# iucario/WorkoutDetector

Hardware: AMD Instinct MI355X
Metric: clips/sec (8x3x224x224 TSM-R50) (higher is better)
Workload: dtype f32; 1 GPU; TSM-R50 8-seg 224x224 12-class inference, batch 32 clips per GPU, f32 NHWC, device-resident input (BASELINE.json configs[1]); clips_per_gpu=32, num_segments=8, height=224, width=224, num_class=12, weights=seeded random init (no trained weights offline), parallelism=single GPU

## Files before the change

workoutdetector_amd/csrc/tsm_conv_rules.h:

```cpp
#pragma once
#include <stdint.h>
#include <string.h>

#if defined(__HIPCC__)
#define TSM_HOST_DEVICE __host__ __device__
#else
#define TSM_HOST_DEVICE
#endif

namespace tsm {

struct ConvParams {
  const float *x;
  const float *w;
  const float *bias;
  const float *res;
  float *y;
  int N, Hi, Wi, C, logC4;
  int Ho, Wo, Cout;
  int stride, pad;
  int Kp;
  int M;
  int relu;
  int T;
  int fold;
  int ntm, ntn;
  int tile;
  int prec;
  const float *x2;
  int C2, Hi2, Wi2, stride2;
  int K1;
  int kseg_len;
  int ksplit;
  int tail_from;
  float *ypart;
  int reverse;
  int pos_major;
};

enum ConvPrec { kPrecF32 = 0, kPrecBf16x3 = 1, kPrecBf16 = 2 };
constexpr int kPrecBlockShift = 4;
constexpr int kPrecPosMajor = 8;

enum ConvTile {
  kTileAuto = 0, kTile128x128 = 1, kTile128x64 = 2, kTile64x64 = 3, kTile32x32 = 4,
  kTile128x128w8 = 5,
  kTile256x256 = 6,
  kTileWs = 7,
  kTile256x256p = 8,
  kNumTiles = 9
};

struct Fused23Params {
  const float *x;
  const float *w2;
  const float *bias2;
  const float *w3f;
  const float *bias3;
  const float *res;
  float *y;
// ... 288 lines not shown
    case kTile256x256p:
      return p.prec == kPrecBf16 && p.Cout % 256 == 0 && p.C % 64 == 0 && !(p.res && p.x2) && (p.pad != 1 || (!p.res && p.T == 0)) &&
             (!p.x2 || (p.K1 % 64 == 0 && p.C2 % 64 == 0)) && (tile == kTile256x256 || (p.Cout <= 2048 && p.Kp >= 128));
    case kTileWs: {
      int tr, tc;
      return conv3x3_ws_valid(p, &tr, &tc) || conv3x3_ws128s2_valid(p, &tr, &tc) || conv3x3_ws128_valid(p, &tr, &tc, nullptr) ||
             conv1x1_ws_valid(p) || conv1x1_wsn_valid(p, n_cu);
    }
    default: return false;
  }
}

enum ConvFamily { kFamInvalid = 0, kFamIgemm, kFamIgemmSeg, kFamBf16_256, kFamBf16_256p, kFamWs3x3, kFamWs128, kFamWs128s2, kFamWs1x1, kFamWsn };

struct ConvRoute {
  int family = kFamInvalid, ks = 0;
  int bm = 0, bn = 0, wgm = 0, wgn = 0;
  bool shift = false, res = false, dual = false, block_shift = false;
  bool pos_major = false;
  int ntm = 0, ntn = 0;
  long tiles = 0;
  unsigned grid = 0;
  int tr = 0, tc = 0, swz = 0;
};

inline bool conv_args_refused(const ConvParams &p, int ks) {
  const int kc = p.prec == kPrecBf16 ? 64 : kBK;
  if (p.Cout % 64 != 0 || p.Kp % kc != 0 || p.M <= 0) return true;
  if (p.logC4 < 0 || p.logC4 > 28 || (1 << p.logC4) * 4 != p.C) return true;
  if (ks != 7 && p.C % kc != 0) return true;
  if (p.T > 0 && ((ks != 1 && ks != 3) || (ks == 3 && p.kseg_len > 0) || p.N % p.T != 0 || p.fold % 4 != 0 ||
                  (p.res && 2 * (int64_t)p.fold > p.Cout) || (p.x2 && 2 * (int64_t)p.fold > p.C2)))
    return true;
  if (p.x2 && (ks != 1 || p.res || p.K1 % kc != 0 || p.C2 % kc != 0 || (int64_t)p.K1 + p.C2 != p.Kp || p.K1 != p.C))
    return true;
  if (p.x2 && (128.0 / ((double)p.Ho * p.Wo) + 4.0) * (double)p.Hi2 * p.Wi2 * p.C2 * 4.0 > 2.0e9) return true;
  if (p.T > 0 && p.res && (128.0 + 2.0 * p.Ho * p.Wo) * p.Cout * 4.0 > 2.0e9) return true;
  if (p.prec != kPrecF32 && p.prec != kPrecBf16x3 && p.prec != kPrecBf16) return true;
  if (p.kseg_len < 0 || (p.kseg_len > 0 && (p.prec != kPrecF32 || p.res || ks == 7))) return true;
  if ((p.ksplit && p.kseg_len <= 0) || p.ksplit < 0 || p.ksplit > 2) return true;
  if (p.prec != kPrecF32 && p.T > 0 && p.fold % 8 != 0) return true;
  if (ks == 7 && (p.C != 4 || (p.prec != kPrecF32 && (p.stride != 2 || p.pad != 3)))) return true;
  if ((128.0 / ((double)p.Ho * p.Wo) + 4.0) * (double)p.Hi * p.Wi * p.C * 4.0 > 2.0e9) return true;
  return (ks != 1 && ks != 3 && ks != 7) || (ks == 7 && p.res);
}

// ... 8 lines not shown
  for (int ky = 0; ky < 3; ++ky)
    for (int kx = 0; kx < 3; ++kx)
      if ((unsigned)(iy0 + ky) < (unsigned)Hi && (unsigned)(ix0 + kx) < (unsigned)Wi) mask |= 1u << (ky * 3 + kx);
  return mask;
}
TSM_HOST_DEVICE inline int next_live_kstep(int kt, unsigned mask, int steps_per_tap, int nk) {
  if (kt < 0 || kt >= nk) return nk;
  const int log_spt = __builtin_ctz((unsigned)steps_per_tap);
  const int tap = kt >> log_spt;
  const unsigned rest = tap < 9 ? (mask & 0x1ffu) >> tap : 0u;
  if (rest & 1u) return kt;
  if (rest == 0u) return nk;
  const int next = (tap + __builtin_ctz(rest)) << log_spt;
  return next < nk ? next : nk;
}
inline bool pos_major_valid(const ConvParams &p, int ks) {
  return p.prec == kPrecF32 && ks == 3 && p.pad == 1 && (p.stride == 1 || p.stride == 2) && p.kseg_len > 0 && p.T == 0 &&
         !p.res && !p.x2 && (p.tile == kTile64x64 || p.tile == kTileAuto) && (p.ksplit == 0 || p.ksplit == 2) &&
         p.N > 0 && p.N % 64 == 0 && p.Ho > 0 && p.Wo > 0 && (int64_t)p.N * p.Ho * p.Wo == p.M &&
         p.C >= kBK && (p.C & (p.C - 1)) == 0 && p.Kp == (int64_t)9 * p.C &&
         (double)p.N * p.Hi * p.Wi * p.C * 4.0 < 2.0e9 && (double)p.M * p.Cout * 4.0 < 2.0e9;
}

inline ConvRoute conv_route(const ConvParams &p, int ks, int n_cu) {
  ConvRoute r, refused;
  if (conv_args_refused(p, ks) || (p.tile != kTileAuto && !conv_tile_valid(p, p.tile, n_cu))) return refused;
  r.ks = ks; r.res = p.res != nullptr; r.dual = p.x2 != nullptr;
  r.shift = !r.res && p.T > 0 && !(ks == 1 && r.dual);
  if (p.tile == kTileAuto) conv_tile_shape(p, &r.bm, &r.bn);
  else conv_tile_dims(p.tile, &r.bm, &r.bn);
  if (p.tile == kTile256x256 || p.tile == kTile256x256p) {
    const bool persistent = p.tile == kTile256x256p;
    if (!(persistent ? conv_bf16_256p_valid(p, ks) : conv_bf16_256_valid(p, ks))) return refused;
    r.family = persistent ? kFamBf16_256p : kFamBf16_256;
    r.wgm = 2; r.wgn = 4;
    r.shift = ks == 1 && p.T > 0;
    r.ntm = (int)(((long)p.M + 255) / 256); r.ntn = p.Cout / 256;
    r.tiles = (long)r.ntm * r.ntn;
    const int slots = n_cu & ~7;
    r.grid = (unsigned)(!persistent || r.tiles < slots || slots < 8 ? r.tiles : slots);
    return r.tiles > 0x7fffffffL ? refused : r;
  }
  if (p.tile == kTileWs) {
    if (ks == 3) {
      r.family = conv3x3_ws128s2_valid(p, &r.tr, &r.tc) ? kFamWs128s2 : conv3x3_ws128_valid(p, &r.tr, &r.tc, &r.swz) ? kFamWs128 :
                 conv3x3_ws_valid(p, &r.tr, &r.tc) ? kFamWs3x3 : kFamInvalid;
// ... 11 lines not shown
      const int pairs = n_cu >> 4 << 3;
      r.grid = 2u * (unsigned)(r.tiles < pairs ? (r.tiles + 7) / 8 * 8 : pairs);
    }
    return r;
  }
  if (p.kseg_len > 0 && r.bm != 32) r.bm = r.bn = 64;
  if (r.bm == 32 && p.prec != kPrecF32) return refused;
  r.wgm = r.bm == 32 ? 1 : r.bm == 128 && r.bn == 128 && p.tile == kTile128x128w8 ? 4 : 2;
  r.wgn = r.bm == 32 ? 1 : 2;
  r.ntm = (int)(((long)p.M + r.bm - 1) / r.bm); r.ntn = p.Cout / r.bn;
  r.tiles = (long)r.ntm * r.ntn;
  long grid = r.tiles;
  if (p.kseg_len > 0) {
    if (r.res || ks == 7 || (r.shift && ks == 3)) return refused;
    if (p.ksplit == 2 && (p.tail_from <= 0 || p.tail_from >= r.tiles || p.tail_from % r.ntn != 0)) return refused;
    r.family = kFamIgemmSeg;
    r.pos_major = p.pos_major != 0 && r.bm == 64 && pos_major_valid(p, ks);
    grid = p.ksplit == 2 ? p.tail_from + (r.tiles - p.tail_from) * conv_num_segments(p) : r.tiles * (p.ksplit ? conv_num_segments(p) : 1);
  } else {
    r.family = kFamIgemm;
  }
  r.block_shift = p.T > 0 && (r.dual || r.res);
  r.grid = (unsigned)grid;
  return grid > 0x7fffffffL ? refused : r;
}

inline bool conv23_ws_valid(int n, int h, int w, int *tr_out = nullptr, int *tc_out = nullptr) {
  int tr, tc;
  return n > 0 && h > 0 && w > 0 && (double)h * w * 512.0 < 2.0e9 && (double)n * h * w < 2.0e9 &&
         ws_tile_geometry(h, w, tr_out ? tr_out : &tr, tc_out ? tc_out : &tc);
}
inline bool bneck_ws_valid(int cin, int n, int h, int w, int T, int fold) {
  return (cin == 256 || cin == 64) && n > 0 && h > 0 && w >= 1 && w <= 64 && (double)h * w * 512.0 * 3.0 < 2.0e9 &&
         (T == 0 || (T > 0 && n % T == 0 && fold == cin / 8));
}
inline bool front_s2_valid(int n, int h, int w, int T, int fold) {
  return n > 0 && h >= 2 && (h & 1) == 0 && w >= 2 && w <= 64 && (double)h * w * 512.0 * 3.0 < 2.0e9 &&
         (T == 0 || (T > 0 && n % T == 0 && fold == 32));
}
inline int conv31_rows(const Conv31Params &p) {
  if (p.K3 == 128 && p.C == 512 && p.N1 == 128) return 256;
  if ((p.K3 == 128 && p.C == 512 && p.N1 == 256) || (p.K3 == 256 && p.C == 1024 && p.N1 == 256)) return 128;
  return 0;
}
inline bool conv31_valid(const Conv31Params &p) {
  const int m = conv31_rows(p);
  if (m == 0) return false;
// ... 7 lines not shown
```

workoutdetector_amd/csrc/tsm_engine.hip:

```cpp
#include <hip/hip_runtime.h>

#include <sys/stat.h>

#include <algorithm>
#include <cerrno>
#include <cmath>
#include <cstdio>
#include <cstdlib>
#include <cstring>
#include <map>
#include <string>
#include <vector>

#include "../../include/tsm_hip.h"
#include "tsm_host_util.h"
#include "tsm_kernels.h"

#ifndef TSM_BUILD_ID
#define TSM_BUILD_ID __DATE__ "/" __TIME__
#endif

namespace {

using namespace tsm_host;
// ... 151 lines not shown
  float *d_in4 = nullptr;
  float *buf[5] = {nullptr, nullptr, nullptr, nullptr, nullptr};
  float *d_pooled = nullptr, *d_logits = nullptr;
  float *d_partial = nullptr;
  size_t partial_elems = 0;
  size_t buf_elems = 0;
  int h1 = 0, w1 = 0, hp = 0, wp = 0;
  hipEvent_t ev0 = nullptr, ev1 = nullptr;
  bool have_time = false;
  std::vector<void *> allocs;
  bool poison = false;
  std::vector<GuardBuf> guards;
  std::map<int, std::vector<int>> tile_cache;
  bool autotune = true;
  bool stem_pool = true;
  bool stem_direct = true;
  bool stem_planar = true;
  std::string tune_path, tune_sig;
  int force_tile = 0, force_code = -1;
  int fuse23 = -1;
  int fuse_block = -1;
  int fuse31 = -1;
  int fuse_front = -1;
  bool pos_major = true;
  int walk = -1;
  int n_cu = 256;
  int timing_left = 0;
  bool timing_only3x3 = false;
  std::vector<std::vector<hipEvent_t>> timing;
  std::vector<hipEvent_t> event_pool;
  std::vector<hipEvent_t> *cur_timing = nullptr;
};

namespace {

int fail(tsm_engine *e, int code, const std::string &msg) {
  if (e) e->err = msg; else g_create_error = msg;
  return code;
}

#define TSM_HIP(e, call)                                                                        \
  do {                                                                                          \
    hipError_t _st = (call);                                                                    \
    if (_st != hipSuccess)                                                                      \
      return fail((e), TSM_ERR_HIP, std::string(#call) + ": " + hipGetErrorString(_st));        \
  } while (0)
// ... 320 lines not shown
  fclose(f);
  return ok;
}

void tune_cache_store(tsm_engine *e, int key, const std::vector<int> &codes) {
  if (e->tune_path.empty()) return;
  std::string line = e->tune_sig + "|" + std::to_string(key) + "|";
  for (size_t i = 0; i < codes.size(); ++i) line += (i ? "," : "") + std::to_string(codes[i]);
  line += "\n";
  if (line.size() >= 4096) return;
  FILE *f = fopen(e->tune_path.c_str(), "a");
  if (!f) return;
  fwrite(line.data(), 1, line.size(), f);
  fclose(f);
}

bool tail_split_from(const tsm::ConvParams &p, int n_cu, size_t partial_elems, int *tail_from) {
  if (p.kseg_len <= 0) return false;
  const long from = tsm_host::tail_split_point(p.M, p.Cout, tsm::conv_num_segments(p), n_cu, partial_elems);
  *tail_from = (int)from;
  return from > 0;
}

hipError_t launch_conv_code(tsm::ConvParams p, int ks, int code, float *partial, size_t partial_elems, int n_cu, hipStream_t s) {
  p.tile = code & kCodeTileMask;
  const bool pos_major = (code & kCodePosMajor) && !(code & kCodeSplitK) && (code & kCodeTileMask) == tsm::kTile64x64 &&
                         tsm::pos_major_valid(p, ks);
  p.pos_major = pos_major ? 1 : 0;
  if ((code & kCodeSplitK) && p.kseg_len > 0 &&
      (size_t)tsm::conv_num_segments(p) * (size_t)p.M * (size_t)p.Cout <= partial_elems) {
    float *y = p.y;
    p.ksplit = 1;
    p.y = partial;
    hipError_t st = tsm::launch_conv(p, ks, s);
    if (st == hipSuccess)
      st = tsm::launch_splitk_reduce(partial, tsm::conv_num_segments(p), p.M, p.Cout, p.bias, nullptr, y, p.relu, s);
    return st;
  }
  if ((code & kCodeTailK) && (code & kCodeTileMask) == tsm::kTile64x64 && p.kseg_len > 0) {
    int tail_from = 0;
    if (tail_split_from(p, n_cu, partial_elems, &tail_from)) {
      float *y = p.y;
      const int mt0 = tail_from / (p.Cout / 64) * 64;
      p.ksplit = 2;
      p.tail_from = tail_from;
      p.ypart = partial;
      hipError_t st = tsm::launch_conv(p, ks, s);
      if (st == hipSuccess && pos_major)
        st = tsm::launch_splitk_reduce_pos(partial, tsm::conv_num_segments(p), mt0, p.M - mt0, p.N, p.Ho * p.Wo, p.Cout, p.bias, y,
                                           p.relu, s);
      else if (st == hipSuccess)
        st = tsm::launch_splitk_reduce(partial, tsm::conv_num_segments(p), p.M - mt0, p.Cout, p.bias, nullptr,
                                       y + (size_t)mt0 * p.Cout, p.relu, s);
      return st;
    }
  }
  return tsm::launch_conv(p, ks, s);
}

int checked_code(const tsm::ConvParams &p, int code, int n_cu) {
  return code > 0 && (code & ~kCodeValid) == 0 && tsm::conv_tile_valid(p, code & kCodeTileMask, n_cu) ? code : 0;
}

struct Tap {
  const float *ptr = nullptr;
  int64_t shape[4] = {0, 0, 0, 0};
  bool hit = false;
};

struct LaunchTimer {
  tsm_engine *e;
  hipStream_t s;
  bool on;
  bool skip;
  LaunchTimer(tsm_engine *e_, hipStream_t s_, bool is3x3)
      : e(e_), s(s_), on(e_->cur_timing != nullptr), skip(e_->timing_only3x3 && !is3x3) { mark(); }
  ~LaunchTimer() { mark(); }
  void mark() {
    if (!on) return;
    if (skip) {
      e->cur_timing->push_back(nullptr);
      return;
    }
    hipEvent_t ev = nullptr;
// ... 175 lines not shown
    int rc = time_best_of(e, s, many, &many_ms);
    if (!rc) rc = time_best_of(e, s, one, &one_ms);
    *wins = one_ms < many_ms;
    return rc;
  }
  int conv(int idx, tsm::ConvParams p, int ks, bool is3x3);
  int run_basic(size_t k, int nn, float *x, float *y, int hh, int ww);
  int run_block(size_t k, const BlockPlan &plan, int nn, float *x, float *y, int hh, int ww);
  int run_nonlocal(size_t k, int nn, float *x, float *z, int hh, int ww);
  int run_mse(size_t k, int nn, int hh, int ww);
  int tune_block(size_t k, int nn, float *x, float *y, int hh, int ww);
};

hipError_t Forward::launch_code(tsm::ConvParams p, int ks, int code) {
  return launch_conv_code(p, ks, code, e->d_partial, e->partial_elems, e->n_cu, s);
}

int Forward::conv(int idx, tsm::ConvParams p, int ks, bool is3x3) {
  p.reverse = next_dir();
  if (!tuning) {
    int code = tiles ? (*tiles)[idx] : 0;
    if (e->force_tile) code = e->force_tile;
    if (e->force_code >= 0) code = e->force_code;
    TSM_LAUNCH_K(e, s, is3x3, launch_code(p, ks, checked_code(p, code, e->n_cu)));
    return TSM_OK;
  }
  std::vector<int> cands;
  if (p.kseg_len > 0) {
    const size_t need = (size_t)tsm::conv_num_segments(p) * p.M * p.Cout;
    const long tiles64 = (long)((p.M + 63) / 64) * (p.Cout / 64);
    for (int t : {(int)tsm::kTile64x64, (int)tsm::kTile32x32}) {
      cands.push_back(t);
      if (need <= e->partial_elems && tiles64 < 4L * e->n_cu) cands.push_back(t | kCodeSplitK);
    }
    int tail_from = 0;
    const bool tail = tail_split_from(p, e->n_cu, e->partial_elems, &tail_from);
    if (tail) cands.push_back((int)tsm::kTile64x64 | kCodeTailK);
    tsm::ConvParams q = p;
    q.tile = tsm::kTile64x64;
    if (e->pos_major && tsm::pos_major_valid(q, ks)) {
      cands.push_back((int)tsm::kTile64x64 | kCodePosMajor);
      if (tail) cands.push_back((int)tsm::kTile64x64 | kCodePosMajor | kCodeTailK);
    }
  } else {
    for (int t = 1; t < tsm::kNumTiles; ++t)
      if (tsm::conv_tile_valid(p, t, e->n_cu)) cands.push_back(t);
  }
  float best_ms = 0.f;
  int best = 0;
  for (int t : cands) {
    float ms = 0.f;
    const int rc = time_best_of(e, s, [&] { return launch_code(p, ks, t); }, &ms);
    if (rc) return rc;
    if (best == 0 || ms < best_ms) {
      best = t;
      best_ms = ms;
    }
  }
  (*tiles)[idx] = best;
  return TSM_OK;
}

int Forward::run_basic(size_t k, int nn, float *x, float *y, int hh, int ww) {
  const Block &blk = e->blocks[k];
  const std::string &name = blk.name;
  const ConvLayer &c1 = e->convs[blk.conv1], &c2 = e->convs[blk.conv2];
  const int T = blk.T, shiftT = e->cfg.is_shift ? T : 0;
  const int ho = conv_out_size(hh, 3, blk.stride), wo = conv_out_size(ww, 3, blk.stride);
  const float *identity = x;
// ... 876 lines not shown
  }
  if (cfg->shift_div <= 0 || (64 % cfg->shift_div) != 0 || (64 / cfg->shift_div) % 4 != 0)
    return fail(nullptr, TSM_ERR_UNSUPPORTED, "shift_div must divide 64 with fold % 4 == 0 (8 or 16... )");
  if (prec_of_dtype(cfg->dtype) < 0)
    return fail(nullptr, TSM_ERR_UNSUPPORTED, "dtype must be TSM_DTYPE_F32, TSM_DTYPE_BF16X3 or TSM_DTYPE_BF16");
  if (cfg->dtype != TSM_DTYPE_F32 && (64 / cfg->shift_div) % 8 != 0)
    return fail(nullptr, TSM_ERR_UNSUPPORTED, "the bf16 formats need fold % 8 == 0 (shift_div <= 8)");
  int ndev = 0;
  hipError_t st = hipGetDeviceCount(&ndev);
  if (st != hipSuccess || ndev <= 0)
    return fail(nullptr, TSM_ERR_HIP, std::string("no HIP device: ") + hipGetErrorString(st));
  if (cfg->device_id < 0 || cfg->device_id >= ndev) return fail(nullptr, TSM_ERR_INVALID_ARG, "bad device_id");
  tsm_engine *e = new tsm_engine();
  e->cfg = *cfg;
  e->prec = prec_of_dtype(cfg->dtype);
  const auto on = [](const char *s) { return atoi(s) != 0; };
  env_read("TSM_AUTOTUNE", &e->autotune, on);
  env_read("TSM_STEM_DIRECT", &e->stem_direct, on);
  env_read("TSM_STEM_POOL", &e->stem_pool, on);
  env_read("TSM_STEM_PLANAR", &e->stem_planar, on);
  env_read("TSM_CONV_TILE", &e->force_tile, tsm::conv_tile_from_name);
  env_read("TSM_CONV_CODE", &e->force_code, atoi);
  env_read("TSM_POS_MAJOR", &e->pos_major, on);
  env_read("TSM_FUSE_CONV23", &e->fuse23, on);
  env_read("TSM_FUSE_BLOCK", &e->fuse_block, on);
  env_read("TSM_FUSE_C3C1", &e->fuse31, on);
  env_read("TSM_FUSE_FRONT", &e->fuse_front, on);
  env_read("TSM_WALK", &e->walk, on);
  env_read("TSM_POISON", &e->poison, on);
  const char *tc = getenv("TSM_TUNE_CACHE");
  if (!tc) e->tune_path = default_tune_cache_path();
  else if (*tc && strcmp(tc, "0") != 0 && strcmp(tc, "off") != 0) e->tune_path = tc;
  build_topology(e);
  st = hipSetDevice(cfg->device_id);
  if (st == hipSuccess) st = hipStreamCreateWithFlags(&e->stream, hipStreamNonBlocking);
  if (st == hipSuccess) st = hipDeviceGetAttribute(&e->n_cu, hipDeviceAttributeMultiprocessorCount, cfg->device_id);
  if (st == hipSuccess) st = hipEventCreate(&e->ev0);
  if (st == hipSuccess) st = hipEventCreate(&e->ev1);
  if (st != hipSuccess) {
    g_create_error = std::string("engine init: ") + hipGetErrorString(st);
    delete e;
    return TSM_ERR_HIP;
  }
  if (!e->tune_path.empty()) {
    hipDeviceProp_t prop;
    e->tune_sig = "abi" + std::to_string(TSM_ABI_VERSION) + " build " TSM_BUILD_ID " " +
                  (hipGetDeviceProperties(&prop, cfg->device_id) == hipSuccess ? std::string(prop.gcnArchName) : "?") +
                  " cu" + std::to_string(e->n_cu) +
                  " T" + std::to_string(cfg->num_segments) + " " + std::to_string(cfg->height) + "x" +
                  std::to_string(cfg->width) + " dtype" + std::to_string(cfg->dtype) + " shift" +
                  std::to_string(cfg->is_shift ? cfg->shift_div : 0) + " fuse" + std::to_string(e->fuse23) + "/" + std::to_string(e->fuse_block) + "/" + std::to_string(e->fuse31) + "/" + std::to_string(e->fuse_front) +
                  " stem" + std::to_string(e->stem_direct ? 1 : 0) +
                  std::to_string(e->stem_pool ? 1 : 0) + std::to_string(e->stem_planar ? 1 : 0);
    e->tune_sig_base = e->tune_sig.size();
  }
  *out = e;
  return TSM_OK;
}

int tsm_set_backbone(tsm_engine *e, int32_t depth) {
  if (int rc = check_before_weights(e, "tsm_set_backbone")) return rc;
  if (int rc = refuse_on_convnext(e, "tsm_set_backbone")) return rc;
  if (!find_backbone(depth)) return fail(e, TSM_ERR_UNSUPPORTED, "depth must be 18, 34 or 50");
  if (find_backbone(depth)->basic && e->width != 64)
    return fail(e, TSM_ERR_UNSUPPORTED, "a BasicBlock backbone (depth 18 / 34) has no bottleneck width: the engine's is " +
                                            std::to_string(e->width));
  if (find_backbone(depth)->basic && e->non_local)
    return fail(e, TSM_ERR_UNSUPPORTED, "non-local blocks need a Bottleneck backbone (depth 50)");
  e->depth = depth;
  e->backbone_set = 1;
  build_topology(e);
  retag_tune_sig(e);
  return TSM_OK;
}

int tsm_set_bottleneck_width(tsm_engine *e, int32_t width_per_group) {
// ... 457 lines not shown
  };
  const float *xin = a->x, *x2in = a->x2, *rin = a->residual;
  float *yout = a->y, *d_x4 = nullptr, *d_ys = nullptr, *d_part = nullptr;
  if (pl.stem) {
    if ((rc = scratch.alloc(&d_x4, "d_x4", n * in_px * 8, in_px * 8))) return rc;
    TSM_HIP(nullptr, tsm::launch_pack_input(a->x, d_x4, n, hi, wi, 0, prec, s));
    xin = d_x4;
  } else if (x3 && (rc = staged(a->x, "d_xs", (size_t)pl.x_elems, in_px * a->cin, &xin))) {
    return rc;
  }
  if (x3) {
    if ((rc = scratch.alloc(&d_ys, "d_ys", out_elems, out_frame, act_bytes))) return rc;
    yout = d_ys;
    if (rin && (rc = staged(rin, "d_rs", out_elems, out_frame, &rin))) return rc;
    if (pl.dual && (rc = staged(x2in, "d_x2s", (size_t)pl.x2_elems, (size_t)a->hi2 * a->wi2 * a->cin2, &x2in))) return rc;
  }
  tsm::ConvParams p = make_params(c, xin, rin, yout, n, hi, wi, a->relu != 0, pl.T, 1, prec);
  p.fold = pl.fold;
  p.reverse = a->reverse != 0;
  if (pl.dual) set_second_source(&p, c2.kp, x2in, a->cin2, a->hi2, a->wi2, a->stride2);
  int dev = 0, n_cu = 256;
  TSM_HIP(nullptr, hipGetDevice(&dev));
  TSM_HIP(nullptr, hipDeviceGetAttribute(&n_cu, hipDeviceAttributeMultiprocessorCount, dev));
  const int code = checked_code(p, a->code > 0 ? a->code & ~kCodeOpSegmented : a->code, n_cu);
  size_t part_elems = 0;
  if ((code & (kCodeSplitK | kCodeTailK)) && p.kseg_len > 0) {
    part_elems = (size_t)tsm::conv_num_segments(p) * p.M * p.Cout;
    if ((rc = scratch.alloc(&d_part, "d_part", part_elems, out_frame))) return rc;
  }
  const char *sd_env = getenv("TSM_STEM_DIRECT");
  hipError_t st;
  if (pl.stem && x3 && cout == 64 && !(sd_env && atoi(sd_env) == 0))
    st = tsm::launch_stem_direct(xin, c.d_w, c.d_b, yout, n, hi, wi, c.kp, a->relu != 0, prec, s);
  else
    st = launch_conv_code(p, a->k, code, d_part, part_elems, n_cu, s);
  if (st == hipSuccess && x3) st = tsm::launch_to_f32(d_ys, a->y, (int64_t)out_elems / 8, prec, s);
  const hipError_t st2 = hipStreamSynchronize(s);
  if (st != hipSuccess) return op_status("launch_conv", st);
  if (st2 != hipSuccess) return fail(nullptr, TSM_ERR_HIP, std::string("conv sync: ") + hipGetErrorString(st2));
  for (int i = 0; i < scratch.n; ++i) {
    std::string msg;
    TSM_HIP(nullptr, guard_verify(scratch.g[i], &msg));
    if (!msg.empty()) return fail(nullptr, TSM_ERR_GUARD, "tsm_conv_op: " + msg);
  }
  return TSM_OK;
}

// ... 228 lines not shown
```

workoutdetector_amd/csrc/tsm_host_util.h:

```cpp
#pragma once
#include <cmath>
#include <cstddef>
#include <cstdint>
#include <cstdio>
#include <cstdlib>
#include <cstring>
#include <string>
#include <vector>

#include "../../include/tsm_hip.h"
#include "tsm_conv_rules.h"

namespace tsm_host {

constexpr float kBnEps = 1e-5f;
using tsm::kPrecF32;
using tsm::kPrecBf16x3;
using tsm::kPrecBf16;

inline int segment_len(int kp, int prec) {
  if (prec != kPrecF32) return 0;
  const int nk = kp / 32;
  if (nk < 32) return 0;
  const int nseg = nk / 16;
// ... 803 lines not shown
    for (int wn = 0; wn < wgn; ++wn)
      for (int kq = 0; kq < nkq; ++kq)
        for (int lane = 0; lane < 64; ++lane) {
          const int n = j * cmid + wn * 32 + (lane & 31), k0 = 16 * kq + 8 * (lane >> 5);
          const size_t base = ((((size_t)j * wgn + wn) * (2 * nkq) + 2 * kq) * 64 + lane) * 8;
          for (int e = 0; e < 8; ++e) {
            const float x = w3p[(size_t)n * cmid + k0 + e];
            const uint16_t hi = f2bf(x);
            o[base + e] = hi;
            o[base + 64 * 8 + e] = f2bf(x - bf2f(hi));
          }
        }
}

constexpr int kCodeTileMask = 0xF;
constexpr int kCodePosMajor = 0x80;
constexpr int kCodeSplitK = 0x100;
constexpr int kCodeTailK = 0x200;
constexpr int kCodeConv23 = 0x400;
constexpr int kCodeBlock = 0x800;
constexpr int kCodeConv31 = 0x1000;
constexpr int kCodeFront = 0x2000;
constexpr int kCodeFused = kCodeConv23 | kCodeBlock | kCodeConv31 | kCodeFront;
constexpr int kCodeValid = kCodeTileMask | kCodePosMajor | kCodeSplitK | kCodeTailK | kCodeFused;
static_assert((kCodeOpSegmented & kCodeValid) == 0, "the per-op segmented bit must stay clear of the engine's code bits");

inline bool parse_tune_line(const char *line, const std::string &want, int num_tiles, std::vector<int> *codes) {
  if (strncmp(line, want.c_str(), want.size()) != 0) return false;
  std::vector<int> got;
  const char *q = line + want.size();
  while (*q && *q != '\n') {
    char *end = nullptr;
    const long v = strtol(q, &end, 10);
    if (end == q) return false;
    if (v < 0 || (v & ~(long)kCodeValid) != 0 || (int)(v & kCodeTileMask) >= num_tiles) return false;
    got.push_back((int)v);
    if (*end == ',') q = end + 1;
    else if (*end == '\n' || *end == 0) q = end;
    else return false;
  }
  if (got.size() != codes->size()) return false;
  *codes = got;
  return true;
}

}
```

workoutdetector_amd/csrc/tsm_igemm.hip:

```cpp
#include "tsm_device.h"

namespace tsm {

template <int BM, int BN, int WGM, int WGN, int KS, bool SHIFT, bool RES, int PREC, bool DUAL = false, bool SEG = false>
__global__ void __launch_bounds__(64 * WGM * WGN, (SEG && BM == 64) ? ((PREC & kPrecBlockShift) ? 4 : 5) : 1)
conv_igemm(const ConvParams p) {
  constexpr bool BSHIFT = (PREC & kPrecBlockShift) != 0;
  constexpr bool POSM = (PREC & kPrecPosMajor) != 0;
  constexpr int PMODE = PREC & ~(kPrecBlockShift | kPrecPosMajor);
  static_assert(!POSM || (SEG && KS == 3 && BM == 64 && BN == 64 && !SHIFT && !RES && !DUAL && !BSHIFT && PMODE == kPrecF32),
                "position-major rows: the segmented fp32 3x3 on 64x64 tiles only (pos_major_valid)");
  static_assert(!BSHIFT || (!SHIFT && !RES), "block placement: a shifted identity (DUAL = false) or a shifted second source");
  constexpr bool RESID = RES || (BSHIFT && !DUAL);
  static_assert(!SEG || (PMODE == kPrecF32 && !RES && WGM * WGN <= 4 && BM == BN && BM <= 64),
                "segmented K accumulation: fp32, 64x64 / 32x32 tiles, no residual (ConvParams::kseg_len)");
  static_assert(WGM * WGN == 4 || WGM * WGN == 1 || WGM * WGN == 8,
                "4 waves per workgroup, 1 (32x32 small-M tiles) or 8 (128x128 with 4 waves per SIMD at 2 workgroups/CU)");
  constexpr int NT = 64 * WGM * WGN;
  constexpr int LRP = NT / 8;
  static_assert(!DUAL || (KS == 1 && !SHIFT && !RES), "K-concatenated second source: plain 1x1 convs only");
  constexpr bool X3 = PMODE == kPrecBf16x3;
  constexpr bool BF = PMODE == kPrecBf16;
  constexpr int EB = BF ? 2 : 4;
  constexpr int KC = 128 / EB;
  static_assert(!SHIFT || KS == 1 || (KS == 3 && !SEG), "the temporal shift is fused into 1x1 and unsegmented 3x3 convs only");
  constexpr int WTM = BM / WGM, WTN = BN / WGN;
  constexpr int TM = WTM / 32, TN = WTN / 32;
  constexpr int APASS = BM / LRP, BPASS = BN / LRP;
  constexpr bool RK = PMODE == kPrecF32 && ((BM == 64 && BN == 64) || (BM == 32 && BN == 32));
  constexpr int NBUF = RK ? 1 : 2;
  constexpr int CLD = BN + 4;
  static_assert(TM >= 1 && TN >= 1, "wave tile must hold at least one 32x32 MFMA tile");
  constexpr int SMEM_FLOATS = NBUF * (BM + BN) * kLds > BM * CLD ? NBUF * (BM + BN) * kLds : BM * CLD;

  __shared__ __attribute__((aligned(16))) float smem[SMEM_FLOATS];

  const int tid = threadIdx.x;
  const int lane = tid & 63;
  const int wave = tid >> 6;
  const int wm = wave / WGN, wn = wave % WGN;
  const int half = lane >> 5, l31 = lane & 31;

  const int bid = blockIdx.x;
  const bool tail_mode = SEG && p.ksplit == 2;
  const bool in_tail = tail_mode && bid >= p.tail_from;
  const int nwg = tail_mode ? p.tail_from : (int)gridDim.x;
  const int q = nwg >> 3, r = nwg & 7, xcd = bid & 7;
  int tile = (xcd < r ? xcd * (q + 1) : r * (q + 1) + (xcd - r) * q) + (bid >> 3);
  if (p.reverse) tile = nwg - 1 - tile;
  int seg = 0;
  if (SEG && p.ksplit == 1) {
    seg = tile / (p.ntm * p.ntn);
    tile -= seg * (p.ntm * p.ntn);
  }
  if (in_tail) {
    const int u = bid - p.tail_from, n_tail = p.ntm * p.ntn - p.tail_from;
    seg = u / n_tail;
    tile = p.tail_from + (u - seg * n_tail);
  }
  const bool split_wg = SEG && (p.ksplit == 1 || in_tail);
  const int tm = tile / p.ntn, tn = tile - tm * p.ntn;
  const int m0 = tm * BM, n0 = tn * BN;

  const int HoWo = p.Ho * p.Wo;
  const int n_first = POSM ? 0 : m0 / HoWo;
  const int frame0 = SHIFT ? (n_first > 0 ? n_first - 1 : 0) : n_first;
  constexpr bool PAIRS = KS == 7 && PMODE != kPrecF32;
  const int wpairs = (p.Wi + 1) >> 1;
  const size_t frame_elems = PAIRS ? (size_t)p.Hi * wpairs * 8 : (size_t)p.Hi * p.Wi * p.C;
  const size_t a_bytes = ((size_t)p.N - frame0) * frame_elems * EB;
  const __amdgpu_buffer_rsrc_t rsrcA = buffer_window(reinterpret_cast<const char *>(p.x) + (size_t)frame0 * frame_elems * EB, a_bytes);
  const __amdgpu_buffer_rsrc_t rsrcB = buffer_fixed(reinterpret_cast<const char *>(p.w) + (size_t)n0 * p.Kp * EB, BN * p.Kp * EB);

  const size_t frame_elems2 = DUAL ? (size_t)p.Hi2 * p.Wi2 * p.C2 : 0;
  const int frame02 = (BSHIFT && DUAL && n_first > 0) ? n_first - 1 : n_first;
  const size_t a2_bytes = DUAL ? ((size_t)p.N - frame02) * frame_elems2 * EB : 0;
  const __amdgpu_buffer_rsrc_t rsrcA2 = buffer_window(reinterpret_cast<const char *>(DUAL ? p.x2 : p.x) + (size_t)frame02 * frame_elems2 * EB, a2_bytes);

  const int lrow = tid >> 3;
  const int chunk = tid & 7;
  const int frame_bytes = (int)(frame_elems * EB);
  unsigned a_off[APASS];
  unsigned a_offp[SHIFT ? APASS : 1], a_offm[SHIFT ? APASS : 1];
  unsigned a_mask[(KS == 3 && !POSM) ? APASS : 1];
// ... 636 lines not shown
  if constexpr (RES && !SHIFT && KS != 7) {
    if (r.block_shift) TSM_LAUNCH_IGEMM_AND_RETURN(TSM_ARM_RES_SHIFT);
  }
  TSM_LAUNCH_IGEMM_AND_RETURN(TSM_ARM_PLAIN);
}

template <int KS, bool SHIFT, bool RES>
static hipError_t launch_conv_ks(const ConvParams &p, const ConvRoute &r, hipStream_t s) {
  if (r.bm == 32) return launch_conv_t<32, 32, 1, 1, KS, SHIFT, RES>(p, r, s);
  if (r.bm == 128 && r.bn == 128 && r.wgm == 4) return launch_conv_t<128, 128, 4, 2, KS, SHIFT, RES>(p, r, s);
  if (r.bm == 128 && r.bn == 128) return launch_conv_t<128, 128, 2, 2, KS, SHIFT, RES>(p, r, s);
  if (r.bm == 128) return launch_conv_t<128, 64, 2, 2, KS, SHIFT, RES>(p, r, s);
  return launch_conv_t<64, 64, 2, 2, KS, SHIFT, RES>(p, r, s);
}

hipError_t launch_conv(const ConvParams &p_in, int ks, hipStream_t s) {
  const bool device = p_in.tile == kTile256x256 || p_in.tile == kTile256x256p || p_in.tile == kTileWs;
  const DeviceInfo *di = device ? &device_info() : nullptr;
  const ConvRoute r = conv_route(p_in, ks, di ? di->n_cu : 0);
  if (r.family == kFamInvalid) return hipErrorInvalidValue;
  if (di && di->status != hipSuccess) return di->status;
  ConvParams p = p_in;
  p.ntm = r.ntm; p.ntn = r.ntn;
  if (r.family == kFamBf16_256 || r.family == kFamBf16_256p) return launch_conv_bf16_256(p, r, s);
  if (r.family >= kFamWs3x3) return launch_conv_ws(p, r, s);
  if (p.ksplit == 2 && !p.ypart) return hipErrorInvalidValue;
  if (ks == 1) return r.res ? launch_conv_ks<1, false, true>(p, r, s) : r.shift ? launch_conv_ks<1, true, false>(p, r, s) : launch_conv_ks<1, false, false>(p, r, s);
  if (ks == 3) return r.res ? launch_conv_ks<3, false, true>(p, r, s) : r.shift ? launch_conv_ks<3, true, false>(p, r, s) : launch_conv_ks<3, false, false>(p, r, s);
  return launch_conv_ks<7, false, false>(p, r, s);
}

__global__ void __launch_bounds__(256) splitk_reduce_kernel(const float *__restrict__ partial, int n_seg, int64_t n4,
                                                            int64_t seg_stride4, int cout4,
                                                            const float *__restrict__ bias, const float *__restrict__ res,
                                                            float *__restrict__ y, int relu) {
  const int64_t stride = (int64_t)gridDim.x * blockDim.x;
  const float floor_ = relu ? 0.f : -INFINITY;
  const f32x4 *p4 = reinterpret_cast<const f32x4 *>(partial);
  for (int64_t i = (int64_t)blockIdx.x * blockDim.x + threadIdx.x; i < n4; i += stride) {
    f32x4 t = p4[i];
    for (int sgm = 1; sgm < n_seg; ++sgm) t += p4[i + sgm * seg_stride4];
    f32x4 v = t + reinterpret_cast<const f32x4 *>(bias)[i % cout4];
    if (res) v += reinterpret_cast<const f32x4 *>(res)[i];
    v[0] = fmaxf(v[0], floor_);
    v[1] = fmaxf(v[1], floor_);
    v[2] = fmaxf(v[2], floor_);
// ... 50 lines not shown
```

workoutdetector_amd/engine.py:

```python
from __future__ import annotations

import ctypes as C
from dataclasses import dataclass
from typing import Dict, List, Mapping, Optional, Sequence

import numpy as np

from . import _lib
from .weights import (BACKBONES, CONVNEXT, CONVNEXT_DEPTHS, CONVNEXT_WIDTHS, DEPTHS, NL_BLOCKS, SHIFT_PLACES, TDN, TDN_FRAMES, WIDTHS,
                      _convnext_depths, _tdn_depths, feature_width, is_convnext, is_mmaction_state_dict, make_state_dict, make_tdn_state_dict,
                      remap_checkpoint_keys, remap_mmaction_keys, remap_tdn_keys, remap_timm_keys, remap_torchvision_keys, tdn_alpha_beta)

CONSENSUS_TYPES = {'avg': 0, 'identity': 1}


@dataclass
class NodeArg:
    name: str
    shape: list
    type: str = 'tensor(float)'


def _as_f32(a) -> np.ndarray:
    return np.ascontiguousarray(np.asarray(a), dtype=np.float32)
# ... 466 lines not shown
        for li, nb in enumerate(blocks, start=1):
            for b in range(nb):
                p = f'layer{li}.{b}'
                if kind == 'basic':
                    names += ([p + '.downsample'] if b == 0 and li > 1 else []) + [p + '.conv1', p + '.conv2']
                else:
                    names += ([p + '.downsample'] if b == 0 else []) + [p + '.conv1', p + '.conv2', p + '.conv3']
                    if self.non_local and (li, b) in NL_BLOCKS:
                        names += [p + '.nl.qkv', p + '.nl.pool', p + '.nl.attn', p + '.nl.W']
            if self.temporal_pool and li == 1:
                names.append('layer2.tpool')
        return names + ['head']

    @property
    def tdn_chunk_clips(self) -> int:
        per_clip = (self.height // 4) * (self.width // 4) * self.num_segments * 1024
        return max(1, min(8, self.max_clips, ((1 << 29) - 1) // per_clip))

    TILE_NAMES = {0: 'heuristic', 1: '128x128', 2: '128x64', 3: '64x64', 4: '32x32', 5: '128x128w8', 6: '256x256', 7: 'ws',
                  8: '256x256p'}

    @classmethod
    def tile_name(cls, code: int) -> str:
        return (cls.TILE_NAMES[code & 15] + ('/pos' if code & 0x80 else '') + ('/splitK' if code & 0x100 else '') + ('/tailK' if code & 0x200 else '') + ('+conv3' if code & 0x400 else '') +
                ('+block' if code & 0x800 else '') + ('+conv1' if code & 0x1000 else '') + ('+conv2' if code & 0x2000 else ''))

    def conv_tiles(self, n_clips: int) -> Dict[str, str]:
        buf = (C.c_int32 * 256)()
        n = C.c_int32()
        _lib.check(self._lib.tsm_conv_tiles(self._h, n_clips, buf, 256, C.byref(n)), self._h)
        if self.tdn_depths:
            names = ['conv1', 'diff.conv1_5'] + [k for k in self.launch_names() if k.startswith(('resnext_layer1.', 'layer'))
                                                 and k.endswith(('.downsample', '.conv1', '.conv2', '.conv3'))]
            assert n.value == len(names)
            return {k: self.tile_name(buf[i]) for i, k in enumerate(names)}
        if self.convnext_depths:
            names = [k for k in self.launch_names() if k == 'stem.conv' or k.endswith(('.downsample', '.fc1', '.fc2'))]
            assert n.value == len(names)
            return {k: self.tile_name(buf[i]) for i, k in enumerate(names)}
        names = [k for k in self.launch_names() if k not in ('pack_input', 'maxpool', 'head', 'layer2.tpool') and not k.endswith(('.nl.pool', '.nl.attn'))]
        assert n.value == len(names)
        return {k: self.tile_name(buf[i]) for i, k in enumerate(names)}

    def set_layer_timing(self, n_forwards: int, only_conv3x3: bool = False) -> None:
        _lib.check(self._lib.tsm_set_layer_timing(self._h, n_forwards, int(only_conv3x3)), self._h)

    def layer_times_ms(self, forward_index: int) -> Dict[str, float]:
# ... 672 lines not shown
```

Before: 1870 clips/s.

## Add XCD-blocked tile ordering and pos-major frame grouping as autotune candidates

Adds a tile-to-workgroup mapping that splits the output tile grid into 2D blocks per XCD, so each XCD's L2 holds only a slice of the weight columns instead of the full weight matrix. It also adds an optional row remap for the pos-major path that interleaves frame groups. Both are new bits in the tuning code. The autotuner adds them as candidates only when a byte model predicts fewer L2 misses. The cost is a more complex index calculation and more autotune candidates.

After: 1867 clips/s. Within noise of the previous version (-0.2%).

```diff
diff --git a/workoutdetector_amd/csrc/tsm_conv_rules.h b/workoutdetector_amd/csrc/tsm_conv_rules.h
--- a/workoutdetector_amd/csrc/tsm_conv_rules.h
+++ b/workoutdetector_amd/csrc/tsm_conv_rules.h
@@ -36,6 +36,8 @@
   float *ypart;
   int reverse;
   int pos_major;
+  int xcd_n;
+  int pm_group;
 };
 
 enum ConvPrec { kPrecF32 = 0, kPrecBf16x3 = 1, kPrecBf16 = 2 };
@@ -370,6 +372,8 @@
   long tiles = 0;
   unsigned grid = 0;
   int tr = 0, tc = 0, swz = 0;
+  int n_whole = 0, xcd_n = 1;
+  bool pm_group = false;
 };
 
 inline bool conv_args_refused(const ConvParams &p, int ks) {
@@ -424,6 +428,53 @@
          (double)p.N * p.Hi * p.Wi * p.C * 4.0 < 2.0e9 && (double)p.M * p.Cout * 4.0 < 2.0e9;
 }
 
+constexpr int kXcds = 8;
+constexpr long kXcdL2Bytes = 4L << 20;
+constexpr long kXcdSlabMaxBytes = kXcdL2Bytes / 8 * 5;
+
+TSM_HOST_DEVICE inline int xcd_tile_contiguous(int bid, int n_whole, int reverse) {
+  const int q = n_whole >> 3, r = n_whole & 7, xcd = bid & 7;
+  const int tile = (xcd < r ? xcd * (q + 1) : r * (q + 1) + (xcd - r) * q) + (bid >> 3);
+  return reverse ? n_whole - 1 - tile : tile;
+}
+TSM_HOST_DEVICE inline bool xcd_blocks_equal(int ntm, int ntn, int n_whole, int xcd_n) {
+  if (xcd_n != 2 && xcd_n != 4 && xcd_n != 8) return false;
+  if (ntm <= 0 || ntn <= 0 || n_whole <= 0 || n_whole % ntn != 0 || ntn % xcd_n != 0) return false;
+  const int rows = n_whole / ntn;
+  return (rows <= ntm || rows % ntm == 0) && rows % (kXcds / xcd_n) == 0;
+}
+TSM_HOST_DEVICE inline int xcd_tile(int bid, int ntm, int ntn, int n_whole, int xcd_n, int reverse) {
+  if (!xcd_blocks_equal(ntm, ntn, n_whole, xcd_n)) return xcd_tile_contiguous(bid, n_whole, reverse);
+  const int xcd = bid & 7, brow = xcd / xcd_n, bcol = xcd - brow * xcd_n;
+  const int bc = ntn / xcd_n, br = n_whole / ntn / (kXcds / xcd_n);
+  int local = bid >> 3;
+  if (reverse) local = br * bc - 1 - local;
+  const int lr = local / bc, lc = local - lr * bc;
+  return (brow * br + lr) * ntn + bcol * bc + lc;
+}
+inline bool xcd_order_valid(int ntm, int ntn, int n_whole, int xcd_n, int cout, int kp, int elem_bytes) {
+  return xcd_blocks_equal(ntm, ntn, n_whole, xcd_n) && (int64_t)(cout / xcd_n) * kp * elem_bytes <= kXcdSlabMaxBytes;
+}
+inline double xcd_order_bytes(double act_bytes, double w_bytes, int xcd_n, long rows, int ntn, int resident_per_xcd) {
+  if (xcd_n > 1) return (double)kXcds * (w_bytes / xcd_n) + act_bytes * xcd_n;
+  long passes = 1;
+  if (w_bytes > (double)kXcdSlabMaxBytes) {
+    const long rows_xcd = (rows + kXcds - 1) / kXcds, cover = resident_per_xcd / (ntn > 0 ? ntn : 1);
+    passes = (rows_xcd + (cover > 0 ? cover : 1) - 1) / (cover > 0 ? cover : 1);
+  }
+  return (double)kXcds * (double)(passes > 0 ? passes : 1) * w_bytes + act_bytes;
+}
+inline int conv_tile_wg_per_cu(int bm, int bn) { return bm == 32 ? 8 : bm == 64 ? 5 : bn == 64 ? 3 : 2; }
+
+TSM_HOST_DEVICE inline int pos_major_group_row(int tm, int rows_whole, int n_frames) {
+  const int g = n_frames >> 6;
+  if (g <= 1) return tm;
+  const int npos = rows_whole / g;
+  if (tm >= npos * g) return tm;
+  const int fg = tm / npos, pos = tm - fg * npos;
+  return pos * g + fg;
+}
+
 inline ConvRoute conv_route(const ConvParams &p, int ks, int n_cu) {
   ConvRoute r, refused;
   if (conv_args_refused(p, ks) || (p.tile != kTileAuto && !conv_tile_valid(p, p.tile, n_cu))) return refused;
@@ -481,7 +532,11 @@
   }
   r.block_shift = p.T > 0 && (r.dual || r.res);
   r.grid = (unsigned)grid;
-  return grid > 0x7fffffffL ? refused : r;
+  if (grid > 0x7fffffffL) return refused;
+  r.n_whole = r.family == kFamIgemmSeg && p.ksplit == 2 ? p.tail_from : (int)grid;
+  if (p.xcd_n > 1 && xcd_order_valid(r.ntm, r.ntn, r.n_whole, p.xcd_n, p.Cout, p.Kp, p.prec == kPrecBf16 ? 2 : 4)) r.xcd_n = p.xcd_n;
+  r.pm_group = r.pos_major && p.pm_group != 0 && p.N >= 128;
+  return r;
 }
 
 inline bool conv23_ws_valid(int n, int h, int w, int *tr_out = nullptr, int *tc_out = nullptr) {
diff --git a/workoutdetector_amd/csrc/tsm_engine.hip b/workoutdetector_amd/csrc/tsm_engine.hip
--- a/workoutdetector_amd/csrc/tsm_engine.hip
+++ b/workoutdetector_amd/csrc/tsm_engine.hip
@@ -197,6 +197,7 @@
   int fuse_block = -1;
   int fuse31 = -1;
   int fuse_front = -1;
+  int xcd_order = 1;
   bool pos_major = true;
   int walk = -1;
   int n_cu = 256;
@@ -563,13 +564,29 @@
   return from > 0;
 }
 
+int apply_code(tsm::ConvParams *p, int ks, int code, size_t partial_elems, int n_cu) {
+  p->tile = code & kCodeTileMask;
+  const bool pos_major = (code & kCodePosMajor) && !(code & kCodeSplitK) && (code & kCodeTileMask) == tsm::kTile64x64 &&
+                         tsm::pos_major_valid(*p, ks);
+  p->pos_major = pos_major ? 1 : 0;
+  p->xcd_n = 1 << ((code & kCodeXcdMask) >> kCodeXcdShift);
+  p->pm_group = pos_major && (code & kCodePosGroup) ? 1 : 0;
+  if ((code & kCodeSplitK) && p->kseg_len > 0 &&
+      (size_t)tsm::conv_num_segments(*p) * (size_t)p->M * (size_t)p->Cout <= partial_elems)
+    return 1;
+  int tail_from = 0;
+  if ((code & kCodeTailK) && (code & kCodeTileMask) == tsm::kTile64x64 && p->kseg_len > 0 &&
+      tail_split_from(*p, n_cu, partial_elems, &tail_from)) {
+    p->tail_from = tail_from;
+    return 2;
+  }
+  return 0;
+}
+
 hipError_t launch_conv_code(tsm::ConvParams p, int ks, int code, float *partial, size_t partial_elems, int n_cu, hipStream_t s) {
-  p.tile = code & kCodeTileMask;
-  const bool pos_major = (code & kCodePosMajor) && !(code & kCodeSplitK) && (code & kCodeTileMask) == tsm::kTile64x64 &&
-                         tsm::pos_major_valid(p, ks);
-  p.pos_major = pos_major ? 1 : 0;
-  if ((code & kCodeSplitK) && p.kseg_len > 0 &&
-      (size_t)tsm::conv_num_segments(p) * (size_t)p.M * (size_t)p.Cout <= partial_elems) {
+  const int form = apply_code(&p, ks, code, partial_elems, n_cu);
+  const bool pos_major = p.pos_major != 0;
+  if (form == 1) {
     float *y = p.y;
     p.ksplit = 1;
     p.y = partial;
@@ -578,29 +595,55 @@
       st = tsm::launch_splitk_reduce(partial, tsm::conv_num_segments(p), p.M, p.Cout, p.bias, nullptr, y, p.relu, s);
     return st;
   }
-  if ((code & kCodeTailK) && (code & kCodeTileMask) == tsm::kTile64x64 && p.kseg_len > 0) {
-    int tail_from = 0;
-    if (tail_split_from(p, n_cu, partial_elems, &tail_from)) {
-      float *y = p.y;
-      const int mt0 = tail_from / (p.Cout / 64) * 64;
-      p.ksplit = 2;
-      p.tail_from = tail_from;
-      p.ypart = partial;
-      hipError_t st = tsm::launch_conv(p, ks, s);
-      if (st == hipSuccess && pos_major)
-        st = tsm::launch_splitk_reduce_pos(partial, tsm::conv_num_segments(p), mt0, p.M - mt0, p.N, p.Ho * p.Wo, p.Cout, p.bias, y,
-                                           p.relu, s);
-      else if (st == hipSuccess)
-        st = tsm::launch_splitk_reduce(partial, tsm::conv_num_segments(p), p.M - mt0, p.Cout, p.bias, nullptr,
-                                       y + (size_t)mt0 * p.Cout, p.relu, s);
-      return st;
-    }
+  if (form == 2) {
+    float *y = p.y;
+    const int mt0 = p.tail_from / (p.Cout / 64) * 64;
+    p.ksplit = 2;
+    p.ypart = partial;
+    hipError_t st = tsm::launch_conv(p, ks, s);
+    if (st == hipSuccess && pos_major)
+      st = tsm::launch_splitk_reduce_pos(partial, tsm::conv_num_segments(p), mt0, p.M - mt0, p.N, p.Ho * p.Wo, p.Cout, p.bias, y,
+                                         p.relu, s);
+    else if (st == hipSuccess)
+      st = tsm::launch_splitk_reduce(partial, tsm::conv_num_segments(p), p.M - mt0, p.Cout, p.bias, nullptr,
+                                     y + (size_t)mt0 * p.Cout, p.relu, s);
+    return st;
   }
   return tsm::launch_conv(p, ks, s);
 }
 
-int checked_code(const tsm::ConvParams &p, int code, int n_cu) {
-  return code > 0 && (code & ~kCodeValid) == 0 && tsm::conv_tile_valid(p, code & kCodeTileMask, n_cu) ? code : 0;
+int checked_code(const tsm::ConvParams &p, int ks, int code, int n_cu, size_t partial_elems) {
+  if (!(code > 0 && (code & ~kCodeValid) == 0 && tsm::conv_tile_valid(p, code & kCodeTileMask, n_cu))) return 0;
+  if (code & (kCodeXcdMask | kCodePosGroup)) {
+    tsm::ConvParams q = p;
+    q.ksplit = apply_code(&q, ks, code, partial_elems, n_cu);
+    const tsm::ConvRoute r = tsm::conv_route(q, ks, n_cu);
+    if (r.xcd_n != q.xcd_n) code &= ~kCodeXcdMask;
+    if (!r.pm_group) code &= ~kCodePosGroup;
+  }
+  return code;
+}
+
+int xcd_code_bits(int xcd_n) { return xcd_n == 2 ? 1 << kCodeXcdShift : xcd_n == 4 ? 2 << kCodeXcdShift : xcd_n == 8 ? 3 << kCodeXcdShift : 0; }
+int parse_xcd_order(const char *s) {
+  const int v = atoi(s);
+  return v == 0 || v == 2 || v == 4 || v == 8 ? v : 1;
+}
+int xcd_order_env() {
+  const char *s = getenv("TSM_XCD_ORDER");
+  return s ? parse_xcd_order(s) : 1;
+}
+bool xcd_order_saves(const tsm::ConvParams &p, int ks, int code, int n_cu, size_t partial_elems) {
+  tsm::ConvParams q = p;
+  q.ksplit = apply_code(&q, ks, code, partial_elems, n_cu);
+  const tsm::ConvRoute r = tsm::conv_route(q, ks, n_cu);
+  if (r.xcd_n <= 1) return false;
+  const double eb = p.prec == tsm::kPrecBf16 ? 2.0 : 4.0;
+  const double act = ((double)p.N * p.Hi * p.Wi * p.C + (p.x2 ? (double)p.N * p.Hi2 * p.Wi2 * p.C2 : 0.0)) * eb;
+  const double w = (double)p.Cout * p.Kp * eb;
+  const long rows = r.n_whole / r.ntn;
+  const int resident = n_cu / tsm::kXcds * tsm::conv_tile_wg_per_cu(r.bm, r.bn);
+  return tsm::xcd_order_bytes(act, w, r.xcd_n, rows, r.ntn, resident) < tsm::xcd_order_bytes(act, w, 1, rows, r.ntn, resident);
 }
 
 struct Tap {
@@ -822,7 +865,8 @@
     int code = tiles ? (*tiles)[idx] : 0;
     if (e->force_tile) code = e->force_tile;
     if (e->force_code >= 0) code = e->force_code;
-    TSM_LAUNCH_K(e, s, is3x3, launch_code(p, ks, checked_code(p, code, e->n_cu)));
+    if (e->xcd_order > 1 && code > 0) code = (code & ~kCodeXcdMask) | xcd_code_bits(e->xcd_order);
+    TSM_LAUNCH_K(e, s, is3x3, launch_code(p, ks, checked_code(p, ks, code, e->n_cu, e->partial_elems)));
     return TSM_OK;
   }
   std::vector<int> cands;
@@ -845,6 +889,27 @@
   } else {
     for (int t = 1; t < tsm::kNumTiles; ++t)
       if (tsm::conv_tile_valid(p, t, e->n_cu)) cands.push_back(t);
+  }
+  if (e->xcd_order != 0) {
+    const auto checked = [&](int c) { return checked_code(p, ks, c, e->n_cu, e->partial_elems); };
+    const size_t n_base = cands.size();
+    for (size_t i = 0; i < n_base; ++i) {
+      const int c = cands[i];
+      const int grouped = checked(c | kCodePosGroup);
+      if (grouped != c && grouped != 0 && e->xcd_order == 1) cands.push_back(grouped);
+      if (e->xcd_order > 1) {
+        const int forced = checked(c | xcd_code_bits(e->xcd_order));
+        if (forced != 0) cands[i] = forced;
+        continue;
+      }
+      for (int xn : {2, 4, 8})
+        for (int base : {c, grouped}) {
+          const int cc = checked(base | xcd_code_bits(xn));
+          if (base != 0 && (cc & kCodeXcdMask) && xcd_order_saves(p, ks, cc, e->n_cu, e->partial_elems) &&
+              std::find(cands.begin(), cands.end(), cc) == cands.end())
+            cands.push_back(cc);
+        }
+    }
   }
   float best_ms = 0.f;
   int best = 0;
@@ -1767,6 +1832,7 @@
   env_read("TSM_CONV_TILE", &e->force_tile, tsm::conv_tile_from_name);
   env_read("TSM_CONV_CODE", &e->force_code, atoi);
   env_read("TSM_POS_MAJOR", &e->pos_major, on);
+  env_read("TSM_XCD_ORDER", &e->xcd_order, parse_xcd_order);
   env_read("TSM_FUSE_CONV23", &e->fuse23, on);
   env_read("TSM_FUSE_BLOCK", &e->fuse_block, on);
   env_read("TSM_FUSE_C3C1", &e->fuse31, on);
@@ -1796,7 +1862,8 @@
                   std::to_string(cfg->width) + " dtype" + std::to_string(cfg->dtype) + " shift" +
                   std::to_string(cfg->is_shift ? cfg->shift_div : 0) + " fuse" + std::to_string(e->fuse23) + "/" + std::to_string(e->fuse_block) + "/" + std::to_string(e->fuse31) + "/" + std::to_string(e->fuse_front) +
                   " stem" + std::to_string(e->stem_direct ? 1 : 0) +
-                  std::to_string(e->stem_pool ? 1 : 0) + std::to_string(e->stem_planar ? 1 : 0);
+                  std::to_string(e->stem_pool ? 1 : 0) + std::to_string(e->stem_planar ? 1 : 0) +
+                  " xcd" + std::to_string(e->xcd_order);
     e->tune_sig_base = e->tune_sig.size();
   }
   *out = e;
@@ -2300,7 +2367,10 @@
   int dev = 0, n_cu = 256;
   TSM_HIP(nullptr, hipGetDevice(&dev));
   TSM_HIP(nullptr, hipDeviceGetAttribute(&n_cu, hipDeviceAttributeMultiprocessorCount, dev));
-  const int code = checked_code(p, a->code > 0 ? a->code & ~kCodeOpSegmented : a->code, n_cu);
+  int code_in = a->code > 0 ? a->code & ~kCodeOpSegmented : a->code;
+  if (const int xn = xcd_order_env(); xn > 1 && code_in > 0 && !(code_in & kCodeXcdMask)) code_in |= xcd_code_bits(xn);
+  const size_t part_cap = p.kseg_len > 0 ? (size_t)tsm::conv_num_segments(p) * p.M * p.Cout : 0;
+  const int code = checked_code(p, a->k, code_in, n_cu, part_cap);
   size_t part_elems = 0;
   if ((code & (kCodeSplitK | kCodeTailK)) && p.kseg_len > 0) {
     part_elems = (size_t)tsm::conv_num_segments(p) * p.M * p.Cout;
diff --git a/workoutdetector_amd/csrc/tsm_host_util.h b/workoutdetector_amd/csrc/tsm_host_util.h
--- a/workoutdetector_amd/csrc/tsm_host_util.h
+++ b/workoutdetector_amd/csrc/tsm_host_util.h
@@ -849,7 +849,10 @@
 constexpr int kCodeConv31 = 0x1000;
 constexpr int kCodeFront = 0x2000;
 constexpr int kCodeFused = kCodeConv23 | kCodeBlock | kCodeConv31 | kCodeFront;
-constexpr int kCodeValid = kCodeTileMask | kCodePosMajor | kCodeSplitK | kCodeTailK | kCodeFused;
+constexpr int kCodeXcdShift = 15;
+constexpr int kCodeXcdMask = 0x18000;
+constexpr int kCodePosGroup = 0x20000;
+constexpr int kCodeValid = kCodeTileMask | kCodeXcdMask | kCodePosGroup | kCodePosMajor | kCodeSplitK | kCodeTailK | kCodeFused;
 static_assert((kCodeOpSegmented & kCodeValid) == 0, "the per-op segmented bit must stay clear of the engine's code bits");
 
 inline bool parse_tune_line(const char *line, const std::string &want, int num_tiles, std::vector<int> *codes) {
diff --git a/workoutdetector_amd/csrc/tsm_igemm.hip b/workoutdetector_amd/csrc/tsm_igemm.hip
--- a/workoutdetector_amd/csrc/tsm_igemm.hip
+++ b/workoutdetector_amd/csrc/tsm_igemm.hip
@@ -45,9 +45,7 @@
   const bool tail_mode = SEG && p.ksplit == 2;
   const bool in_tail = tail_mode && bid >= p.tail_from;
   const int nwg = tail_mode ? p.tail_from : (int)gridDim.x;
-  const int q = nwg >> 3, r = nwg & 7, xcd = bid & 7;
-  int tile = (xcd < r ? xcd * (q + 1) : r * (q + 1) + (xcd - r) * q) + (bid >> 3);
-  if (p.reverse) tile = nwg - 1 - tile;
+  int tile = xcd_tile(bid, p.ntm, p.ntn, nwg, p.xcd_n, p.reverse);
   int seg = 0;
   if (SEG && p.ksplit == 1) {
     seg = tile / (p.ntm * p.ntn);
@@ -59,7 +57,11 @@
     tile = p.tail_from + (u - seg * n_tail);
   }
   const bool split_wg = SEG && (p.ksplit == 1 || in_tail);
-  const int tm = tile / p.ntn, tn = tile - tm * p.ntn;
+  int tm = tile / p.ntn;
+  const int tn = tile - tm * p.ntn;
+  if constexpr (POSM) {
+    if (p.pm_group && !in_tail) tm = pos_major_group_row(tm, nwg / p.ntn, p.N);
+  }
   const int m0 = tm * BM, n0 = tn * BN;
 
   const int HoWo = p.Ho * p.Wo;
@@ -742,6 +744,7 @@
   if (di && di->status != hipSuccess) return di->status;
   ConvParams p = p_in;
   p.ntm = r.ntm; p.ntn = r.ntn;
+  p.xcd_n = r.xcd_n; p.pm_group = r.pm_group ? 1 : 0;
   if (r.family == kFamBf16_256 || r.family == kFamBf16_256p) return launch_conv_bf16_256(p, r, s);
   if (r.family >= kFamWs3x3) return launch_conv_ws(p, r, s);
   if (p.ksplit == 2 && !p.ypart) return hipErrorInvalidValue;
diff --git a/workoutdetector_amd/engine.py b/workoutdetector_amd/engine.py
--- a/workoutdetector_amd/engine.py
+++ b/workoutdetector_amd/engine.py
@@ -512,7 +512,8 @@
 
     @classmethod
     def tile_name(cls, code: int) -> str:
-        return (cls.TILE_NAMES[code & 15] + ('/pos' if code & 0x80 else '') + ('/splitK' if code & 0x100 else '') + ('/tailK' if code & 0x200 else '') + ('+conv3' if code & 0x400 else '') +
+        order = ('/fg' if code & 0x20000 else '') + ('/xn%d' % (1 << ((code >> 15) & 3)) if code & 0x18000 else '')
+        return (cls.TILE_NAMES[code & 15] + ('/pos' if code & 0x80 else '') + ('/splitK' if code & 0x100 else '') + ('/tailK' if code & 0x200 else '') + order + ('+conv3' if code & 0x400 else '') +
                 ('+block' if code & 0x800 else '') + ('+conv1' if code & 0x1000 else '') + ('+conv2' if code & 0x2000 else ''))
 
     def conv_tiles(self, n_clips: int) -> Dict[str, str]:
```
